# EryiXie/PlaneRecNet

Hardware: AMD Instinct MI355X
Metric: img/s fwd+bwd @480×640 ResNet101-DCN, 1/2/4/8 MI355X + roofline % (higher is better)
Workload: dtype f32 (tensors and accumulation fp32; plain GEMMs and the tap-walked 4x4/s2, 1x1/s2 and sub-pixel convolutions >= 300 tiles: 2xfp16-piece split MFMA, fp32 accumulate; fp32-only rate in fp32_only_run)

## Files before the change

include/prn.h:

```cpp
#ifndef PRN_H
#define PRN_H
#include <stdint.h>
#ifdef __cplusplus
extern "C" {
#endif

#define PRN_BN_SPLITS 32

int prn_version(void);
const char* prn_last_error(void);

enum { PRN_IN_ZERO = 0, PRN_IN_REFLECT = 1, PRN_IN_UP2_REFLECT = 2, PRN_IN_DILATED = 3, PRN_IN_UP2_PHASE = 4,
       PRN_IN_EMBED1 = 5  };
enum { PRN_EPI_NONE = 0, PRN_EPI_RELU = 1, PRN_EPI_SIGMOID = 2 };

enum { PRN_SPLIT_OFF = 0, PRN_SPLIT_PLAN = 1, PRN_SPLIT_ALWAYS = 2 };
enum { PRN_PIECES_BF16 = 0, PRN_PIECES_F16 = 16 };
typedef struct prn_gemm_opts {
  int32_t split_mode;
  int32_t split_kind;
  int32_t split_products;
  int32_t split_min_tiles;
  float split_min_gflop;
  int32_t wgrad_wgs;
// ... 48 lines not shown
typedef struct prn_flip_item {
  const float* src;
  float* dst;
  int M, C, KH, KW;
  int64_t first;
} prn_flip_item;
int prn_weight_flip_transpose_batched(const prn_flip_item* items_dev, int n_items, int64_t total_blocks, void* stream);

int64_t prn_winograd_tiles(int B, int H, int W);
typedef struct prn_winograd_item {
  const float* src;
  float* u;
  float* ut;
  int M, C;
  int64_t first;
} prn_winograd_item;
int prn_winograd_weights_batched(const prn_winograd_item* items_dev, int n_items, int64_t total_blocks, void* stream);
int prn_winograd_input(const float* x, float* V, int B, int C, int H, int W, int in_mode, void* stream);
int64_t prn_gemm_batched_ws_bytes(int M, int C, int P, int nb, const prn_gemm_opts* opts);
int prn_gemm_batched(int M, int C, int P, int nb, const float* U, const void* u_images, const float* V, float* Y, void* ws, const prn_gemm_opts* opts,
                     void* stream);
int prn_winograd_output(const float* Y, const float* bias, const float* addend, float* y, int B, int M, int H, int W, int epilogue, void* stream);
int prn_winograd_output_bn_fwd(const float* Yt, float* x_out, float* stats, const float* gamma, const float* beta, float* y, float* running_mean,
                               float* running_var, int B, int M, int H, int W, float eps, float momentum, int relu, void* stream);
int prn_winograd_output_bn_bwd(const float* Yt, const float* x, const float* stats, const float* gamma, const float* beta, float* dx, float* dgamma,
                               float* dbeta, int B, int M, int H, int W, int relu, void* stream);
int64_t prn_winograd_wgrad_ws_bytes(int B, int C, int H, int W, int M, const prn_gemm_opts* opts);
int prn_winograd_dy(const float* dy, float* Y, int B, int M, int H, int W, void* stream);
int prn_gemm_batched_nt_splits(int M, int C, int P, int nb, const prn_gemm_opts* opts);
int prn_gemm_batched_nt_kind(int M, int C, int P, int nb, const prn_gemm_opts* opts);
int prn_gemm_batched_nt(int M, int C, int P, int nb, const float* A, const float* Bm, float* ws, const prn_gemm_opts* opts, void* stream);
int prn_winograd_dw(const float* partials, float* dw, int M, int C, int splits, void* stream);
int prn_conv3x3_winograd_wgrad(const float* x, const float* dy, float* dw, void* ws, int B, int C, int H, int W, int M, int in_mode, const prn_gemm_opts* opts,
                               void* stream, int phase);
int prn_conv3x3_winograd_wgrad_v(const float* V, const float* dy, float* dw, void* ws, int B, int C, int H, int W, int M, const prn_gemm_opts* opts, void* stream);
int64_t prn_winograd_tiles_ragged(const prn_ragged* rg, int B);
int64_t prn_conv3x3_winograd_ragged_ws_bytes(const prn_ragged* rg, int B, int C, int M, const prn_gemm_opts* opts);
int prn_conv3x3_winograd_ragged(const float* x, const float* U, const void* u_images, const float* bias, const float* addend, float* y, void* ws,
                                const prn_ragged* rg, int B, int C, int M, int epilogue, const prn_gemm_opts* opts, void* stream);
int64_t prn_winograd_wgrad_ragged_ws_bytes(const prn_ragged* rg, int B, int C, int M, const prn_gemm_opts* opts);
int prn_conv3x3_winograd_wgrad_ragged(const float* x, const float* dy, float* dw, void* ws, const prn_ragged* rg, int B, int C, int M, const prn_gemm_opts* opts,
                                      void* stream);
int64_t prn_conv3x3_winograd_ws_bytes(int B, int C, int H, int W, int M, const prn_gemm_opts* opts);
int prn_conv3x3_winograd(const float* x, const float* U, const void* u_images, const float* bias, const float* addend, float* y, void* ws, int B, int C, int H,
                         int W, int M, int in_mode, int epilogue, const prn_gemm_opts* opts, void* stream);

int64_t prn_conv2d_wgrad_ws_bytes(const prn_conv_desc* d);
int prn_conv2d_wgrad_kernel_kind(const prn_conv_desc* d, int G);
int prn_conv2d_wgrad(const prn_conv_desc* d, const float* x, const float* dy, float* dw, void* ws, void* stream);
#define PRN_WGRAD_GROUP_MAX 16
int64_t prn_conv2d_wgrad_grouped_ws_bytes(const prn_conv_desc* d, int G);
int prn_conv2d_wgrad_grouped(const prn_conv_desc* d, int G, const float* const* x, const float* const* dy, float* dw, void* ws, void* stream);
int prn_conv2d_wgrad_phase(const prn_conv_desc* d, const float* x, const float* dy, float* dw, void* ws, void* stream, int phase);

int prn_up2_phase_weights(const float* w, float* wp, int M, int C, void* stream);
int prn_up2_dgrad_weights(const float* w, float* kd, int M, int C, void* stream);
int prn_replicate_fold(const float* dp, float* dx, int B, int C, int H, int W, void* stream);
int prn_space_to_depth2(const float* in, float* out, int B, int C, int H, int W, void* stream);
int prn_up2_wgrad_combine(const float* dwp, float* dw, int M, int C, void* stream);

int prn_pad_fold(const float* dp, float* dx, int B, int C, int H, int W, int up2, void* stream);
int prn_pad_fold_pitched(const float* dp, float* dx, int B, int C, int H, int W, int pitch, void* stream);

int prn_channel_sum(const float* x, float* out, double* ws, int B, int C, int HW, void* stream);

int prn_dcn_sample(const float* x, const float* om, float* cols, int B, int C, int H, int W, int Ho, int Wo,
                   int stride, float max_offset, void* stream);
int64_t prn_dcn_sample_bwd_ws_bytes(int B, int C, int H, int W, int Ho, int Wo);
int prn_dcn_sample_bwd(const float* x, const float* om, const float* dcols, float* dx, float* d_om, void* ws,
                       int B, int C, int H, int W, int Ho, int Wo, int stride, float max_offset, void* stream);

typedef struct prn_dcn_desc {
  int32_t B, C, H, W;
  int32_t M;
  int32_t stride, pad;
  int32_t Ho, Wo;
  int32_t raw;
  float max_offset;
  int32_t epilogue;
  prn_gemm_opts opts;
} prn_dcn_desc;
int64_t prn_dcnv2_table_bytes(const prn_dcn_desc* d);
int prn_dcnv2_table(const prn_dcn_desc* d, const float* offset, const float* mask, void* table, void* stream);
int64_t prn_dcnv2_fwd_ws_bytes(const prn_dcn_desc* d);
int prn_dcnv2_fwd(const prn_dcn_desc* d, const float* x, const void* table, const float* w, const float* bias, float* y, void* ws, void* stream);
int prn_dcnv2_fwd_phase(const prn_dcn_desc* d, const float* x, const void* table, const float* w, const float* bias, float* y, void* ws, void* stream,
                        int phase);
int64_t prn_dcnv2_bwd_weight_ws_bytes(const prn_dcn_desc* d);
int prn_dcnv2_bwd_weight(const prn_dcn_desc* d, const float* x, const void* table, const float* dy, float* dw, void* ws, void* stream);
int prn_dcnv2_bwd_weight_phase(const prn_dcn_desc* d, const float* x, const void* table, const float* dy, float* dw, void* ws, void* stream, int phase);
int64_t prn_dcnv2_bwd_ws_bytes(const prn_dcn_desc* d);
int prn_dcnv2_bwd_input(const prn_dcn_desc* d, const float* dy, const float* wt, const void* wt_images, const float* offset, const float* mask, float* dx,
                        void* ws, void* stream);
int prn_dcnv2_bwd_input_phase(const prn_dcn_desc* d, const float* dy, const float* wt, const void* wt_images, const float* offset, const float* mask,
                              float* dx, void* ws, void* stream, int phase);
int prn_dcnv2_bwd_offset_mask(const prn_dcn_desc* d, const float* x, const float* offset, const float* mask, float* d_offset, float* d_mask,
                              void* ws, void* stream);

int prn_bn_stats(const float* x, float* stats, float* running_mean, float* running_var, double* ws,
                 int B, int C, int HW, float eps, float momentum, void* stream);
int prn_bn_apply(const float* x, const float* stats, const float* gamma, const float* beta, const float* residual,
                 float* y, int B, int C, int HW, int relu, void* stream);
int prn_bn_kernel_kind(int B, int HW);
int prn_bn_train_fwd(const float* x, float* stats, const float* gamma, const float* beta, const float* residual, float* y,
                     float* running_mean, float* running_var, double* ws, int B, int C, int HW, float eps, float momentum,
                     int relu, void* stream);
// ... 188 lines not shown
```

planerecnet_amd/_lib.py:

```python
import ctypes
import os

_HERE = os.path.dirname(os.path.abspath(__file__))
LIB_PATH = os.environ.get("PRN_LIB") or os.path.join(_HERE, "libprn_hip.so")

c_int, c_float, c_void_p, c_i64 = ctypes.c_int, ctypes.c_float, ctypes.c_void_p, ctypes.c_int64


class GemmOpts(ctypes.Structure):
    _fields_ = [("split_mode", ctypes.c_int32), ("split_kind", ctypes.c_int32), ("split_products", ctypes.c_int32), ("split_min_tiles", ctypes.c_int32),
                ("split_min_gflop", ctypes.c_float), ("wgrad_wgs", ctypes.c_int32), ("wgrad_target", ctypes.c_int32), ("wgrad_split", ctypes.c_int32)]

    def key(self):
        return (self.split_mode, self.split_kind, self.split_products, self.split_min_tiles, self.split_min_gflop, self.wgrad_wgs, self.wgrad_target, self.wgrad_split)


SPLIT_OFF, SPLIT_PLAN, SPLIT_ALWAYS = 0, 1, 2
PIECES_BF16, PIECES_F16 = 0, 16


class ConvDesc(ctypes.Structure):
    _fields_ = [(n, ctypes.c_int32) for n in
                ("B", "C", "H", "W", "M", "KH", "KW", "stride", "pad", "Ho", "Wo", "in_mode", "dil", "epilogue", "ystride", "yH", "yW", "reserved")] + [
                    ("opts", GemmOpts)]
# ... 27 lines not shown
P = c_void_p
_DP = ctypes.POINTER(ConvDesc)
_OP = ctypes.POINTER(GemmOpts)
SIGNATURES = {
    "prn_version": (c_int, []),
    "prn_last_error": (ctypes.c_char_p, []),
    "prn_conv2d_fwd_ws_bytes": (c_i64, [_DP]),
    "prn_conv2d_kernel_kind": (c_int, [_DP]),
    "prn_conv2d_fwd_partials": (c_int, [_DP, ctypes.POINTER(c_i64)]),
    "prn_gemm_opts_default": (None, [_OP]),
    "prn_gemm_pipe": (c_int, [c_int, c_int, c_int, c_int, c_int, _OP]),
    "prn_split_images_bytes": (c_i64, [c_int, c_int, c_int]),
    "prn_split_prepare": (c_int, [P, P, c_int, c_int, c_int, c_int, P]),
    "prn_split_prepare_batched": (c_int, [P, c_int, c_i64, c_i64, c_int, P]),
    "prn_conv2d_fwd": (c_int, [_DP, P, P, P, P, P, P, P]),
    "prn_conv2d_fwd_ragged": (c_int, [_DP, P, P, P, P, P, P, P]),
    "prn_conv2d_wgrad_ragged_ws_bytes": (c_i64, [_DP, P]),
    "prn_conv2d_wgrad_ragged": (c_int, [_DP, P, P, P, P, P, P]),
    "prn_gn_relu_fwd_ragged": (c_int, [P, P, P, P, P, c_int, c_int, c_int, P, c_int, c_float, P]),
    "prn_gn_relu_bwd_ragged": (c_int, [P, P, P, P, P, P, P, P, c_int, c_int, c_int, P, c_int, P]),
    "prn_conv2d_fwd_phase": (c_int, [_DP, P, P, P, P, P, P, P, c_int]),
    "prn_conv2d_fwd_counted": (c_int, [_DP, P, P, P, P, P, P, P, P, P, c_int]),
    "prn_conv2d_wgrad_phase": (c_int, [_DP, P, P, P, P, P, c_int]),
    "prn_weight_flip_transpose": (c_int, [P, P, c_int, c_int, c_int, c_int, P]),
    "prn_weight_flip_transpose_batched": (c_int, [P, c_int, c_i64, P]),
    "prn_winograd_tiles": (c_i64, [c_int, c_int, c_int]),
    "prn_winograd_weights_batched": (c_int, [P, c_int, c_i64, P]),
    "prn_winograd_input": (c_int, [P, P, c_int, c_int, c_int, c_int, c_int, P]),
    "prn_gemm_batched_ws_bytes": (c_i64, [c_int, c_int, c_int, c_int, _OP]),
    "prn_gemm_batched": (c_int, [c_int, c_int, c_int, c_int, P, P, P, P, P, _OP, P]),
    "prn_winograd_output": (c_int, [P, P, P, P, c_int, c_int, c_int, c_int, c_int, P]),
    "prn_winograd_output_bn_fwd": (c_int, [P] * 8 + [c_int] * 4 + [c_float, c_float, c_int, P]),
    "prn_winograd_output_bn_bwd": (c_int, [P] * 8 + [c_int] * 5 + [P]),
    "prn_winograd_wgrad_ws_bytes": (c_i64, [c_int] * 5 + [_OP]),
    "prn_winograd_dy": (c_int, [P, P, c_int, c_int, c_int, c_int, P]),
    "prn_gemm_batched_nt_splits": (c_int, [c_int] * 4 + [_OP]),
    "prn_gemm_batched_nt_kind": (c_int, [c_int] * 4 + [_OP]),
    "prn_conv2d_wgrad_kernel_kind": (c_int, [_DP, c_int]),
    "prn_gemm_batched_nt": (c_int, [c_int, c_int, c_int, c_int, P, P, P, _OP, P]),
    "prn_winograd_dw": (c_int, [P, P, c_int, c_int, c_int, P]),
    "prn_conv3x3_winograd_wgrad": (c_int, [P, P, P, P, c_int, c_int, c_int, c_int, c_int, c_int, _OP, P, c_int]),
    "prn_winograd_tiles_ragged": (c_i64, [P, c_int]),
    "prn_conv3x3_winograd_ragged_ws_bytes": (c_i64, [P, c_int, c_int, c_int, _OP]),
    "prn_conv3x3_winograd_ragged": (c_int, [P, P, P, P, P, P, P, P, c_int, c_int, c_int, c_int, _OP, P]),
    "prn_winograd_wgrad_ragged_ws_bytes": (c_i64, [P, c_int, c_int, c_int, _OP]),
    "prn_conv3x3_winograd_wgrad_ragged": (c_int, [P, P, P, P, P, c_int, c_int, c_int, _OP, P]),
    "prn_conv3x3_winograd_wgrad_v": (c_int, [P, P, P, P, c_int, c_int, c_int, c_int, c_int, _OP, P]),
    "prn_conv3x3_winograd_ws_bytes": (c_i64, [c_int] * 5 + [_OP]),
    "prn_conv3x3_winograd": (c_int, [P, P, P, P, P, P, P, c_int, c_int, c_int, c_int, c_int, c_int, c_int, _OP, P]),
    "prn_conv2d_wgrad_ws_bytes": (c_i64, [_DP]),
    "prn_conv2d_wgrad_grouped_ws_bytes": (c_i64, [_DP, c_int]),
    "prn_conv2d_wgrad_grouped": (c_int, [_DP, c_int, P, P, P, P, P]),
    "prn_conv2d_wgrad": (c_int, [_DP, P, P, P, P, P]),
    "prn_pad_fold": (c_int, [P, P, c_int, c_int, c_int, c_int, c_int, P]),
    "prn_pad_fold_pitched": (c_int, [P, P, c_int, c_int, c_int, c_int, c_int, P]),
    "prn_up2_phase_weights": (c_int, [P, P, c_int, c_int, P]),
    "prn_up2_dgrad_weights": (c_int, [P, P, c_int, c_int, P]),
    "prn_up2_wgrad_combine": (c_int, [P, P, c_int, c_int, P]),
    "prn_space_to_depth2": (c_int, [P, P, c_int, c_int, c_int, c_int, P]),
    "prn_replicate_fold": (c_int, [P, P, c_int, c_int, c_int, c_int, P]),
    "prn_channel_sum": (c_int, [P, P, P, c_int, c_int, c_int, P]),
    "prn_dcn_sample": (c_int, [P, P, P] + [c_int] * 7 + [c_float, P]),
    "prn_dcn_sample_bwd_ws_bytes": (c_i64, [c_int] * 6),
    "prn_dcn_sample_bwd": (c_int, [P, P, P, P, P, P] + [c_int] * 7 + [c_float, P]),
    "prn_dcnv2_table_bytes": (c_i64, [P]),
    "prn_dcnv2_table": (c_int, [P, P, P, P, P]),
    "prn_dcnv2_fwd_ws_bytes": (c_i64, [P]),
    "prn_dcnv2_fwd": (c_int, [P] * 8),
    "prn_dcnv2_fwd_phase": (c_int, [P] * 8 + [c_int]),
    "prn_dcnv2_bwd_weight_ws_bytes": (c_i64, [P]),
    "prn_dcnv2_bwd_weight": (c_int, [P] * 7),
    "prn_dcnv2_bwd_weight_phase": (c_int, [P] * 7 + [c_int]),
    "prn_dcnv2_bwd_ws_bytes": (c_i64, [P]),
    "prn_dcnv2_bwd_input": (c_int, [P] * 9),
    "prn_dcnv2_bwd_input_phase": (c_int, [P] * 9 + [c_int]),
    "prn_bn_kernel_kind": (c_int, [c_int, c_int]),
    "prn_dcnv2_bwd_offset_mask": (c_int, [P] * 8),
    "prn_plane_prior_ws_bytes": (c_i64, [c_int] * 6 + [_OP]),
    "prn_plane_prior_fwd": (c_int, [P] * 7 + [c_int] * 6 + [_OP, P]),
    "prn_plane_prior_fwd_phase": (c_int, [P] * 7 + [c_int] * 6 + [_OP, P, c_int]),
    "prn_plane_prior_wgrad_ws_bytes": (c_i64, [c_int] * 5 + [_OP]),
    "prn_plane_prior_wgrad": (c_int, [P] * 4 + [c_int] * 5 + [_OP, P]),
    "prn_fpn_level_ws_bytes": (c_i64, [c_int] * 8 + [_OP]),
    "prn_fpn_level_fwd": (c_int, [P, P, P, P, c_int, c_int, P, P, P, P, P, P] + [c_int] * 6 + [_OP, P]),
    "prn_frame_to_input": (c_int, [P] + [c_int] * 6 + [P, P, c_int, P, P, P]),
    "prn_mask_loss_ws_floats": (c_int, [c_int]),
    "prn_mask_loss_fwd": (c_int, [P] * 9 + [c_int, c_int, c_int, c_float, c_float, P]),
    "prn_mask_loss_bwd": (c_int, [P] * 8 + [c_int, c_int, P]),
    "prn_vnl_triplets": (c_int, [P] * 12 + [c_int, c_int, c_int, c_float, P]),
    "prn_vnl_scatter": (c_int, [P] * 5 + [c_int, c_int, P]),
    "prn_depth_metrics_ws_doubles": (c_int, []),
    "prn_depth_metrics": (c_int, [P, P, P, P, c_i64, c_float, c_float, P]),
    "prn_vnl_trim_key": (c_int, [P, P, P, P, c_int, P]),
    "prn_vnl_trim_fwd": (c_int, [P, P, P, P, P, P, P, c_int, c_int, c_int, P, P, P, P, P, P]),
    "prn_vnl_trim_ws_bytes": (c_i64, [c_int]),
    "prn_vnl_trim_bwd": (c_int, [P, P, P, P, P, P, P, c_int, c_int, P, P]),
    "prn_loss_ws_doubles": (c_int, [c_int]),
    "prn_focal_sum_fwd": (c_int, [P, P, P, P, c_i64, c_int, c_float, c_float, P]),
    "prn_focal_sum_bwd": (c_int, [P, P, P, P, c_i64, c_int, c_float, c_float, P]),
    "prn_rmse_log_fwd": (c_int, [P, P, P, P, P, c_int, c_int, c_float, c_float, P]),
    "prn_rmse_log_bwd": (c_int, [P, P, P, P, P, c_int, c_int, c_float, c_float, P]),
    "prn_gt_segments": (c_i64, [c_int, c_int]),
    "prn_gt_mask_stats": (c_int, [P, P, c_int, c_int, c_int, c_int, P, P, P, P]),
    "prn_gt_quarter_masks": (c_int, [P, P, c_int, c_int, c_int, P]),
    "prn_gt_sample_triplets": (c_int, [P, P, c_int, c_int, c_int, c_int, P, P, P, P, P, ctypes.c_uint64, ctypes.c_uint64, c_i64, P, P]),
    "prn_adam_chunk_elems": (c_int, []),
# ... 73 lines not shown
```

planerecnet_amd/losses.py:

```python
import collections
import os
import threading

import numpy as np
import torch
import torch.nn.functional as F
from torch import nn

from . import ops
from .config import cfg
from .funcs import center_of_mass, quarter_mask_u8


def _pin(x):
    return x.pin_memory()


class Targets:
    __slots__ = ("B", "cell_ids", "cell_gidx", "cell_inv", "cells_unique", "n_pos", "n_pos_dev", "pos_img", "ins_labels", "cate_labels", "num_ins", "vnl", "lava_adj", "lava_gsum",
                 "ready")


LOSS_STREAMS = bool(int(os.environ.get("PRN_LOSS_STREAMS", "0")))

# ... 108 lines not shown
                "cell_inv": pin(torch.from_numpy(cell_inv)) if cell_mult > 1 else None,
                "cells_unique": cell_mult <= 2,
                "cell_ids": pin(torch.from_numpy(np.concatenate(cell_ids))), "pos_img": pin(torch.from_numpy(np.repeat(np.arange(B), n_pos))),
                "ins_labels": pin(torch.cat(ins_labels, 0)),
                "cate_labels": pin(torch.cat([r for lv in range(L) for r in cate_rows[lv]])),
                "vnl": (self.vnl.prepare_host(host, (H, W)) if cfg.use_plane_loss else None) if with_vnl else "deferred"}

    @torch.no_grad()
    def upload(self, h, gt_depths, device):
        t = Targets()
        t.ready = None
        t.B, t.n_pos, t.num_ins = h["B"], h["n_pos"], h["num_ins"]
        up = lambda x: x.to(device, non_blocking=True)
        t.cell_ids = list(up(h["cell_ids"]).split(h["n_pos"]))
        t.cell_gidx, t.cells_unique = up(h["cell_gidx"]), h["cells_unique"]
        t.cell_inv = up(h["cell_inv"]) if h["cell_inv"] is not None else None
        t.n_pos_dev = up(h["n_pos_f"])
        t.pos_img, t.ins_labels, t.cate_labels = up(h["pos_img"]), up(h["ins_labels"]), up(h["cate_labels"])
        t.vnl = self.vnl.upload(h["vnl"], device) if h["vnl"] is not None else None
        t.lava_gsum = t.lava_adj = None
        if cfg.use_lava_loss:
            B, (H, W), (fh, fw) = h["B"], h["hw"], h["feat"]
            if gt_depths.is_cuda and gt_depths.dtype == torch.float32 and LAVA_GT_KERNEL:
                gd = gt_depths.contiguous()
                grad = torch.empty_like(gd)
                ops.check(ops.lib.prn_lava_gt_weights(ops._p(gd), ops._p(grad), B, H, W, float(self.depth_resolution), ops._stream()), "prn_lava_gt_weights")
                t.lava_gsum = ops.channel_sum(grad.view(1, B, H, W))
            else:
                grad = sobel_sq(gt_depths) / gt_depths.clamp(min=self.depth_resolution) ** 2
                grad = grad.clamp(max=1e-2)
                grad = torch.where(grad < 1e-4, torch.zeros_like(grad), grad)
                t.lava_gsum = grad.flatten(1).sum(1)
            adj = torch.empty(B, 1, fh, fw, device=device, dtype=torch.float32)
            ops.check(ops.lib.prn_resize_bilinear_bwd(ops._p(grad.contiguous()), ops._p(adj), B, fh, fw, H, W, ops._stream()), "prn_resize_bilinear_bwd")
            t.lava_adj = adj
        return t

    def prepare(self, gt_instances, gt_depths, device, mask_feat_size=None):
        return self.upload(self.prepare_host(gt_instances, tuple(gt_depths.shape[-2:]), mask_feat_size), gt_depths, device)

    def forward(self, net, mask_preds, cate_preds, kernel_preds, depth_preds, gt_instances, gt_depths, targets=None):
        dev = mask_preds.device
        B = mask_preds.shape[0]
        fh, fw = mask_preds.shape[-2:]
        t = targets if targets is not None else self.prepare(gt_instances, gt_depths, dev, (fh, fw))
        if getattr(t, "ready", None) is not None:
            torch.cuda.current_stream().wait_event(t.ready)
            t.ready = None
        E = kernel_preds[0].shape[1]

        def instance_terms():
            out = {}
            flat_k = torch.cat([k.reshape(B, E, -1) for k in kernel_preds], 2)
            preds = []
            per_image = torch.split(mask_preds, 1)
            if t.cells_unique and sum(t.n_pos) > 0:
                rows = flat_k.transpose(1, 2).reshape(B * flat_k.shape[2], E).index_select(0, t.cell_gidx)
                if t.cell_inv is not None:
                    rows = rows.index_select(0, t.cell_inv)
                w_img = [r.reshape(-1, E, 1, 1) for r in torch.split(rows, t.n_pos)]
            else:
                flat_kb = flat_k.unbind(0)
                w_img = [flat_kb[b][:, t.cell_ids[b]].t().reshape(t.n_pos[b], E, 1, 1).contiguous() if t.n_pos[b] else None for b in range(B)]
            for b in range(B):
                if t.n_pos[b] == 0:
                    continue
                preds.append(ops.conv2d(per_image[b], w_img[b]).view(t.n_pos[b], fh, fw))
            logits = torch.cat(preds, 0)
            if FUSED_LOSS and logits.is_cuda and logits.shape[0] > 0 and (fh * fw) % 4 == 0 and B <= 64:
                lava = cfg.use_lava_loss
                ins, lav = _MaskLoss.apply(logits, t.ins_labels, t.pos_img, t.lava_adj if lava else None, t.lava_gsum if lava else None,
                                           t.n_pos_dev if lava else None, float(self.ins_loss_weight), float(self.lava_loss_weight))
                out["ins"] = ins
                if lava:
                    out["lav"] = lav
                return out
            ins_sig = torch.sigmoid(logits)
            out["ins"] = dice_loss(ins_sig, t.ins_labels).mean() * self.ins_loss_weight
            if cfg.use_lava_loss:
                seg, npos = t.pos_img, t.n_pos_dev
                num = torch.zeros(B, device=dev, dtype=ins_sig.dtype).index_add_(0, seg, (ins_sig * t.lava_adj[seg, 0]).flatten(1).sum(1))
                ok = (t.lava_gsum > 0) & (npos > 0)
                per_img = torch.where(ok, num / (t.lava_gsum * npos).clamp(min=1e-30), torch.zeros_like(num))
                out["lav"] = per_img.sum() / ok.sum().clamp(min=1) * self.lava_loss_weight
            return out

        def category_term():
            flat_pred = torch.cat([c.permute(0, 2, 3, 1).reshape(-1, self.num_classes) for c in cate_preds])
            if FUSED_LOSS and FUSED_CAT_DPT and flat_pred.is_cuda:
                return {"cat": self.conf_loss_weight * _FocalSum.apply(flat_pred, t.cate_labels, self.focal_loss_alpha, self.focal_loss_gamma) / (t.num_ins + 1)}
            onehot = F.one_hot(t.cate_labels, self.num_classes + 1)[:, : self.num_classes].to(flat_pred.dtype)
            return {"cat": self.conf_loss_weight * sigmoid_focal_sum(flat_pred, onehot, self.focal_loss_alpha, self.focal_loss_gamma) / (t.num_ins + 1)}

        def depth_terms():
            dp = ops.resize_bilinear(depth_preds, (2 * depth_preds.shape[2], 2 * depth_preds.shape[3]))
            if FUSED_LOSS and FUSED_CAT_DPT and dp.is_cuda:
                out = {"dpt": self.depth_loss_weight * _RmseLog.apply(dp, gt_depths, cfg.dataset.min_depth, 1e-9)}
            else:
                out = {"dpt": self.depth_loss_weight * rmse_log(dp, gt_depths, gt_depths > cfg.dataset.min_depth)}
            if cfg.use_plane_loss:
                out["pln"] = self.vnl.batched(dp, gt_depths, t.vnl).mean() * self.pln_loss_weight
            return out

        parts = ops.run_branches([instance_terms, category_term, depth_terms]) if (LOSS_STREAMS and mask_preds.is_cuda) else \
            [instance_terms(), category_term(), depth_terms()]
        losses = {}
        for part in parts:
            losses.update(part)
        if all(k in losses for k in ("ins", "cat", "dpt", "pln", "lav")):
            losses = {k: losses[k] for k in ("ins", "cat", "dpt", "pln", "lav")}
        return losses


FUSED_CAT_DPT = bool(int(os.environ.get("PRN_FUSED_CAT_DPT", "1")))
FUSED_LOSS = bool(int(os.environ.get("PRN_FUSED_LOSS", "1")))


class _MaskLoss(torch.autograd.Function):

    @staticmethod
    def forward(ctx, logits, labels, pos_img, adj, gsum, npos, w_ins, w_lav):
        logits, labels = logits.contiguous(), labels.contiguous()
        P, HW = logits.shape[0], logits[0].numel()
        B = adj.shape[0] if adj is not None else 1
        dev = logits.device
        out = torch.empty(2, device=dev, dtype=torch.float32)
        coef = torch.empty(P, 3, device=dev, dtype=torch.float32)
        ws = torch.empty(ops.lib.prn_mask_loss_ws_floats(P), device=dev, dtype=torch.float32)
        adj_c = adj.contiguous() if adj is not None else None
        ops.check(ops.lib.prn_mask_loss_fwd(ops._p(logits), ops._p(labels), ops._p(adj_c), ops._p(pos_img), ops._p(gsum), ops._p(npos), ops._p(out),
                                            ops._p(coef), ops._p(ws), P, HW, B, w_ins, w_lav, ops._stream()), "prn_mask_loss_fwd")
        ctx.save_for_backward(logits, labels, pos_img, adj_c, coef)
        ins, lav = out.unbind(0)
        return ins, lav

    @staticmethod
    def backward(ctx, g_ins, g_lav):
        logits, labels, pos_img, adj, coef = ctx.saved_tensors
        dz = torch.empty_like(logits)
        g_ins = None if g_ins is None else g_ins.contiguous().float()
        g_lav = None if g_lav is None else g_lav.contiguous().float()
        ops.check(ops.lib.prn_mask_loss_bwd(ops._p(logits), ops._p(labels), ops._p(adj), ops._p(pos_img), ops._p(coef), ops._p(g_ins), ops._p(g_lav),
                                            ops._p(dz), logits.shape[0], logits[0].numel(), ops._stream()), "prn_mask_loss_bwd")
        return dz, None, None, None, None, None, None, None


def dice_loss(p, t):
    p = p.reshape(p.shape[0], -1)
    t = t.reshape(t.shape[0], -1).float()
    return 1 - 2 * (p * t).sum(1) / ((p * p).sum(1) + 0.001 + (t * t).sum(1) + 0.001)


def sigmoid_focal_sum(x, t, alpha, gamma):
    p = torch.sigmoid(x)
    ce = F.binary_cross_entropy_with_logits(x, t, reduction="none")
    p_t = p * t + (1 - p) * (1 - t)
    loss = ce * (1 - p_t) ** gamma
    if alpha >= 0:
        loss = (alpha * t + (1 - alpha) * (1 - t)) * loss
    return loss.sum()


def rmse_log(pred, gt, valid, clamp=1e-9):
    n = pred.shape[0]
    l1 = (torch.log(pred.reshape(n, -1).clamp(min=clamp)) - torch.log(gt.reshape(n, -1).clamp(min=clamp))).abs().mul(valid.reshape(n, -1))
    return torch.sqrt((l1 ** 2).sum(1) / valid.reshape(n, -1).sum(1)).mean()
# ... 590 lines not shown
```

planerecnet_amd/ops.py:

```python
import ctypes

import os
import threading
import weakref

import torch

from . import _lib, profiling
from ._lib import ConvDesc, GemmOpts, IN_ZERO, IN_REFLECT, IN_UP2_REFLECT, IN_DILATED, IN_UP2_PHASE, IN_EMBED1, EPI_NONE, EPI_RELU, EPI_SIGMOID, lib, check


_SIDE = {}
WGRAD_ASYNC = bool(int(os.environ.get("PRN_WGRAD_ASYNC", "0")))


WGRAD_WGS_ASYNC = os.environ.get("PRN_WGRAD_WGS_ASYNC", "512")


_POLICY = {"split_mode": int(os.environ.get("PRN_SPLIT_GEMM", "1")),
           "kind": _lib.PIECES_BF16 if os.environ.get("PRN_SPLIT_KIND", "f16") == "bf16" else _lib.PIECES_F16,
           "products": int(os.environ.get("PRN_SPLIT16_PRODUCTS", "3")),
           "min_gflop": float(os.environ.get("PRN_SPLIT_MIN_GFLOP", "4.0")),
           "min_tiles": int(os.environ.get("PRN_SPLIT_MIN_TILES", os.environ.get("PRN_SPLIT_MIN_TILES_EVAL", "300"))),
           "wgrad_wgs": int(os.environ.get("PRN_WGRAD_WGS", "0") or 0),
# ... 993 lines not shown


class _ConvUp2(torch.autograd.Function):

    @staticmethod
    def forward(ctx, x, w, bias):
        _dev(x, w, bias)
        bias_param = bias
        x, w, bias = _c(x), _c(w), _c(bias)
        B, C, H, W = x.shape
        M = w.shape[0]
        assert w.shape[1:] == (C, 3, 3), (x.shape, w.shape)
        wp = torch.empty(4, M, C, 2, 2, device=x.device, dtype=torch.float32)
        check(lib.prn_up2_phase_weights(_p(w), _p(wp), M, C, _stream()), "prn_up2_phase_weights")
        y = conv_fwd_raw(x, wp, bias, None, M, 2, 1, 0, 2 * H, 2 * W, IN_UP2_PHASE)
        ctx.save_for_backward(x, w)
        ctx.has_bias = bias is not None
        ctx.bias = bias_param
        return y

    @staticmethod
    def backward(ctx, dy):
        x, w = ctx.saved_tensors
        dy = _c(dy)
        B, C, H, W = x.shape
        M = w.shape[0]
        dx = dw = db = None
        if ctx.needs_input_grad[0]:
            kd = torch.empty(C, M, 4, 4, device=x.device, dtype=torch.float32)
            check(lib.prn_up2_dgrad_weights(_p(w), _p(kd), M, C, _stream()), "prn_up2_dgrad_weights")
            dp = conv_fwd_raw(dy, kd, None, None, C, 4, 2, 3, H + 2, W + 2)
            dx = torch.empty_like(x)
            check(lib.prn_replicate_fold(_p(dp), _p(dx), B, C, H, W, _stream()), "prn_replicate_fold")
        def wgrad():
            dyp = torch.empty(4, B, M, H, W, device=x.device, dtype=torch.float32)
            check(lib.prn_space_to_depth2(_p(dy), _p(dyp), B, M, H, W, _stream()), "prn_space_to_depth2")
            dwp = conv_wgrad_raw(x, dyp, M, 2, 1, 0, IN_UP2_PHASE)
            dwo = torch.empty_like(w)
            check(lib.prn_up2_wgrad_combine(_p(dwp), _p(dwo), M, C, _stream()), "prn_up2_wgrad_combine")
            if getattr(_TLS, "side", None) is not None:
                _HELD.append((dyp, dwp))
            return dwo
        if _defer(ctx.needs_input_grad[1], w):
            _deferred_wgrad(w, (x, dy), wgrad, fast=True)
        elif ctx.needs_input_grad[1]:
            dw = wgrad()
        db = _bias_grad(ctx.has_bias and ctx.needs_input_grad[2], ctx.bias, dy)
        return dx, dw, db


UP2_SUBPIXEL = bool(int(os.environ.get("PRN_UP2_SUBPIXEL", "1")))


def conv2d(x, w, bias=None, stride=1, pad=0, in_mode=IN_ZERO, epilogue=EPI_NONE, addend=None):
    if in_mode == IN_UP2_REFLECT and UP2_SUBPIXEL and epilogue == EPI_NONE and addend is None and x.shape[2] > 1 and x.shape[3] > 1:
        return _ConvUp2.apply(x, w, bias)
    return _Conv2d.apply(x, w, bias, addend, stride, pad, in_mode, epilogue, False)


_UP2_PHASE = {}


def conv_up2_inference(x, w, bias=None, relu=False):
    _dev(x, w, bias)
    x, w, bias = _c(x), _c(w), _c(bias)
    B, C, H, W = x.shape
    M = w.shape[0]
    assert w.shape[1:] == (C, 3, 3), (x.shape, w.shape)
    if not (UP2_SUBPIXEL and H > 1 and W > 1):
        return conv2d(x, w, bias, 1, 1, IN_UP2_REFLECT, EPI_RELU if relu else EPI_NONE)
    e = _UP2_PHASE.get(w.data_ptr())
    if e is None or e[0]() is not w or e[1] != w._version:
        wp = torch.empty(4, M, C, 2, 2, device=x.device, dtype=torch.float32)
        check(lib.prn_up2_phase_weights(_p(w), _p(wp), M, C, _stream()), "prn_up2_phase_weights")
        ptr = w.data_ptr()
        e = _UP2_PHASE[ptr] = (weakref.ref(w), w._version, wp)
        weakref.finalize(w, lambda p=ptr, r=e[0]: _UP2_PHASE.pop(p, None) if (_UP2_PHASE.get(p) or (None,))[0] is r else None)
    return conv_fwd_raw(x, e[2], bias, None, M, 2, 1, 0, 2 * H, 2 * W, IN_UP2_PHASE, 1, EPI_RELU if relu else EPI_NONE)


def conv2d_fork(x, w, bias=None, stride=1, pad=0, in_mode=IN_ZERO, epilogue=EPI_NONE, addend=None):
    return _Conv2d.apply(x, w, bias, addend, stride, pad, in_mode, epilogue, True)


_DCN = {}


def _dcn_desc(B, C, H, W, M, stride, pad, raw, max_offset, epi=EPI_NONE):
    oe = _opts_entry("colgrad" in SPLIT_SKIP)
    key = (B, C, H, W, M, stride, pad, raw, float(max_offset), epi, oe[2])
    e = _DCN.get(key)
    if e is None:
        Ho, Wo = (H + 2 * pad - 3) // stride + 1, (W + 2 * pad - 3) // stride + 1
        d = _lib.DcnDesc(B, C, H, W, M, stride, pad, Ho, Wo, int(raw), float(max_offset), epi, oe[0])
        ref = ctypes.byref(d)
        sizes = [lib.prn_dcnv2_table_bytes(ref), lib.prn_dcnv2_fwd_ws_bytes(ref), lib.prn_dcnv2_bwd_weight_ws_bytes(ref), lib.prn_dcnv2_bwd_ws_bytes(ref)]
        if min(sizes) < 0:
            raise RuntimeError(lib.prn_last_error().decode())
        e = _DCN[key] = (d, ref, sizes[0], sizes[1], sizes[2], sizes[3])
    return e


def _f32(nbytes, dev):
    return torch.empty(max(nbytes // 4, 1), device=dev, dtype=torch.float32)


# ... 685 lines not shown
```

Before: 193.8.

## Batch per-image mask dynamic convolutions into one ragged grouped GEMM kernel

Replaces the per-image loop of 1x1 conv2d calls that apply predicted instance kernels to mask features with a single ragged grouped GEMM. New HIP kernels cover forward, dgrad and a split-K wgrad with a reduce pass, reading a per-image row/block table from kernel arguments, so there is one launch per pass instead of one per image plus a cat. It uses plain fp32 MFMA 32x32x2 rather than the split fp16 path, and falls back to the old loop when the plan helper rejects the shapes.

```diff
diff --git a/include/prn.h b/include/prn.h
--- a/include/prn.h
+++ b/include/prn.h
@@ -124,6 +124,13 @@
 int64_t prn_conv2d_wgrad_grouped_ws_bytes(const prn_conv_desc* d, int G);
 int prn_conv2d_wgrad_grouped(const prn_conv_desc* d, int G, const float* const* x, const float* const* dy, float* dw, void* ws, void* stream);
 int prn_conv2d_wgrad_phase(const prn_conv_desc* d, const float* x, const float* dy, float* dw, void* ws, void* stream, int phase);
+
+#define PRN_DYNCONV_MAX_IMAGES 32
+int prn_dynconv_fwd(const float* feat, const float* rows, float* logits, int B, int E, int HW, const int* n_rows, const int* splits, void* stream);
+int prn_dynconv_dgrad(const float* rows, const float* dlogits, float* dfeat, int B, int E, int HW, const int* n_rows, const int* splits, void* stream);
+int64_t prn_dynconv_wgrad_ws_bytes(int B, int E, const int* n_rows, const int* splits);
+int prn_dynconv_wgrad(const float* dlogits, const float* feat, float* drows, void* ws, int B, int E, int HW, const int* n_rows, const int* splits,
+                      void* stream, int phase);
 
 int prn_up2_phase_weights(const float* w, float* wp, int M, int C, void* stream);
 int prn_up2_dgrad_weights(const float* w, float* kd, int M, int C, void* stream);
diff --git a/planerecnet_amd/_lib.py b/planerecnet_amd/_lib.py
--- a/planerecnet_amd/_lib.py
+++ b/planerecnet_amd/_lib.py
@@ -103,6 +103,10 @@
     "prn_conv2d_wgrad_grouped_ws_bytes": (c_i64, [_DP, c_int]),
     "prn_conv2d_wgrad_grouped": (c_int, [_DP, c_int, P, P, P, P, P]),
     "prn_conv2d_wgrad": (c_int, [_DP, P, P, P, P, P]),
+    "prn_dynconv_fwd": (c_int, [P, P, P, c_int, c_int, c_int, P, P, P]),
+    "prn_dynconv_dgrad": (c_int, [P, P, P, c_int, c_int, c_int, P, P, P]),
+    "prn_dynconv_wgrad_ws_bytes": (c_i64, [c_int, c_int, P, P]),
+    "prn_dynconv_wgrad": (c_int, [P, P, P, P, c_int, c_int, c_int, P, P, P, c_int]),
     "prn_pad_fold": (c_int, [P, P, c_int, c_int, c_int, c_int, c_int, P]),
     "prn_pad_fold_pitched": (c_int, [P, P, c_int, c_int, c_int, c_int, c_int, P]),
     "prn_up2_phase_weights": (c_int, [P, P, c_int, c_int, P]),
diff --git a/planerecnet_amd/csrc/prn_dynconv.hip b/planerecnet_amd/csrc/prn_dynconv.hip
--- /dev/null
+++ b/planerecnet_amd/csrc/prn_dynconv.hip
@@ -0,0 +1,292 @@
+#include <stddef.h>
+#include "prn_common.h"
+
+typedef float f32x16 __attribute__((ext_vector_type(16)));
+
+namespace {
+
+constexpr int MAXB = PRN_DYNCONV_MAX_IMAGES;
+struct Tab {
+  int nimg;
+  int row0[MAXB + 1];
+  int blk0[MAXB + 1];
+  int splits[MAXB];
+  int wso[MAXB + 1];
+};
+struct DynArgs {
+  const float* a; const float* b; float* out;
+  int E, HW;
+  Tab tab;
+};
+__device__ __forceinline__ int tab_read(size_t member_offset, int i) {
+  typedef __attribute__((address_space(4))) const int* kptr;
+  kptr base = (kptr)__builtin_amdgcn_kernarg_segment_ptr();
+  return base[(offsetof(DynArgs, tab) + member_offset) / 4 + i];
+}
+#define TAB(member, i) tab_read(offsetof(Tab, member), i)
+
+__device__ __forceinline__ int find_image(int nimg, int bid) {
+  int img = 0;
+  for (int t = 1; t < nimg; ++t)
+    if (bid >= TAB(blk0, t)) img = t;
+  return img;
+}
+
+enum { DYN_FWD = 0, DYN_DGRAD = 1, DYN_WGRAD = 2 };
+
+template <int MODE>
+__global__ __launch_bounds__(256) void dynconv_kernel(DynArgs a) {
+  constexpr int BK = 16, LD = BK + 1, NE = BK / 4;
+  constexpr bool A_KFAST = MODE != DYN_DGRAD;
+  constexpr bool B_KFAST = MODE == DYN_WGRAD;
+  __shared__ float As[2][64 * LD];
+  __shared__ float Bs[2][B_KFAST ? 64 * LD : BK * 64];
+  const int tid = threadIdx.x, lane = tid & 63, wave = tid >> 6;
+  const int wm = wave >> 1, wn = wave & 1;
+  const int bid = blockIdx.x;
+  const int img = find_image(a.tab.nimg, bid);
+  const int r0 = TAB(row0, img), n = TAB(row0, img + 1) - r0, S = TAB(splits, img);
+  const int lid = bid - TAB(blk0, img);
+  const int E = a.E, HW = a.HW;
+
+  int m0, j0, Mlim, Jlim, K, split = 0;
+  if (MODE == DYN_FWD) {
+    const int tm = (n + 63) >> 6;
+    m0 = (lid % tm) * 64; j0 = (lid / tm) * 64; Mlim = n; Jlim = HW; K = E;
+  } else if (MODE == DYN_DGRAD) {
+    const int tm = (E + 63) >> 6;
+    m0 = (lid % tm) * 64; j0 = (lid / tm) * 64; Mlim = E; Jlim = HW; K = n;
+  } else {
+    const int tm = (n + 63) >> 6, nt = tm * ((E + 63) >> 6);
+    const int tile = lid % nt;
+    split = lid / nt;
+    m0 = (tile % tm) * 64; j0 = (tile / tm) * 64; Mlim = n; Jlim = E; K = HW;
+  }
+  const int T = (K + 15) >> 4;
+  const int kt_begin = MODE == DYN_WGRAD ? (int)((int64_t)split * T / S) : 0, kt_end = MODE == DYN_WGRAD ? (int)((int64_t)(split + 1) * T / S) : T;
+  const bool rows_here = m0 + wm * 32 < Mlim;
+
+  const int ak = A_KFAST ? (tid & 15) : (tid >> 6), am = A_KFAST ? (tid >> 4) : (tid & 63);
+  const int bk = B_KFAST ? (tid & 15) : (tid >> 6), bj = B_KFAST ? (tid >> 4) : (tid & 63);
+  const float* ap; const float* bp;
+  int a_ms, a_ks, b_js, b_ks;
+  if (MODE == DYN_FWD) {
+    ap = a.a + (size_t)r0 * E; a_ms = E; a_ks = 1;
+    bp = a.b + (size_t)img * E * HW; b_js = 1; b_ks = HW;
+  } else if (MODE == DYN_DGRAD) {
+    ap = a.a + (size_t)r0 * E; a_ms = 1; a_ks = E;
+    bp = a.b + (size_t)r0 * HW; b_js = 1; b_ks = HW;
+  } else {
+    ap = a.a + (size_t)r0 * HW; a_ms = HW; a_ks = 1;
+    bp = a.b + (size_t)img * E * HW; b_js = HW; b_ks = 1;
+  }
+
+  float ra[NE], rb[NE];
+  auto load_slice = [&](int kt) {
+    const int k0 = kt * 16, kend = kt < kt_end ? K : 0;
+#pragma unroll
+    for (int i = 0; i < NE; ++i) {
+      const int m = m0 + am + (A_KFAST ? 16 * i : 0), k = k0 + ak + (A_KFAST ? 0 : 4 * i);
+      const bool ok = m < Mlim && k < kend;
+      ra[i] = ok ? ap[(size_t)m * a_ms + (size_t)k * a_ks] : 0.f;
+    }
+#pragma unroll
+    for (int i = 0; i < NE; ++i) {
+      const int j = j0 + bj + (B_KFAST ? 16 * i : 0), k = k0 + bk + (B_KFAST ? 0 : 4 * i);
+      const bool ok = j < Jlim && k < kend;
+      rb[i] = ok ? bp[(size_t)j * b_js + (size_t)k * b_ks] : 0.f;
+    }
+  };
+  auto store_slice = [&](int buf) {
+#pragma unroll
+    for (int i = 0; i < NE; ++i) As[buf][(am + (A_KFAST ? 16 * i : 0)) * LD + ak + (A_KFAST ? 0 : 4 * i)] = ra[i];
+#pragma unroll
+    for (int i = 0; i < NE; ++i) {
+      if (B_KFAST) Bs[buf][(bj + 16 * i) * LD + bk] = rb[i];
+      else Bs[buf][(bk + 4 * i) * 64 + bj] = rb[i];
+    }
+  };
+  f32x16 acc, tot;
+#pragma unroll
+  for (int r = 0; r < 16; ++r) { acc[r] = 0.f; tot[r] = 0.f; }
+  auto mma_slice = [&](int buf) {
+    if (!rows_here) return;
+#pragma unroll
+    for (int kk = 0; kk < BK / 2; ++kk) {
+      const int k = kk * 2 + (lane >> 5);
+      const float av = As[buf][(wm * 32 + (lane & 31)) * LD + k];
+      const float bv = B_KFAST ? Bs[buf][(wn * 32 + (lane & 31)) * LD + k] : Bs[buf][k * 64 + wn * 32 + (lane & 31)];
+      acc = __builtin_amdgcn_mfma_f32_32x32x2f32(av, bv, acc, 0, 0, 0);
+    }
+  };
+
+  const bool fold = MODE != DYN_WGRAD && S > 1;
+  int sp = 0, bnd = fold ? (int)((int64_t)T / S) : -1;
+  while (fold && bnd <= 0 && sp < S - 1) { ++sp; bnd = (int)((int64_t)(sp + 1) * T / S); }
+  load_slice(kt_begin);
+  int buf = 0;
+  for (int kt = kt_begin; kt < kt_end; ++kt) {
+    store_slice(buf);
+    __syncthreads();
+    load_slice(kt + 1);
+    mma_slice(buf);
+    buf ^= 1;
+    if (fold && kt + 1 == bnd) {
+#pragma unroll
+      for (int r = 0; r < 16; ++r) { tot[r] += acc[r]; acc[r] = 0.f; }
+      do { ++sp; bnd = (int)((int64_t)(sp + 1) * T / S); } while (bnd <= kt + 1 && sp < S - 1);
+    }
+  }
+  if (fold) acc = tot;
+  float* outp;
+  int ldo;
+  if (MODE == DYN_WGRAD) {
+    outp = a.out + (size_t)TAB(wso, img) + (size_t)split * n * E;
+    ldo = E;
+  } else {
+    outp = MODE == DYN_FWD ? a.out + (size_t)r0 * HW : a.out + (size_t)img * E * HW;
+    ldo = HW;
+  }
+  const int j = j0 + wn * 32 + (lane & 31);
+  if (j >= Jlim) return;
+#pragma unroll
+  for (int r = 0; r < 16; ++r) {
+    const int m = m0 + wm * 32 + (r & 3) + 8 * (r >> 2) + 4 * (lane >> 5);
+    if (m < Mlim) outp[(size_t)m * ldo + j] = acc[r];
+  }
+}
+
+__global__ __launch_bounds__(256) void dynconv_reduce_kernel(DynArgs a) {
+  __shared__ float sm[4][64];
+  const int bid = blockIdx.x;
+  const int img = find_image(a.tab.nimg, bid);
+  const int r0 = TAB(row0, img), n = TAB(row0, img + 1) - r0, splits = TAB(splits, img);
+  const int64_t cnt = (int64_t)n * a.E;
+  const float* ws = a.a + (size_t)TAB(wso, img);
+  const int e = threadIdx.x & 63, g = threadIdx.x >> 6;
+  const int64_t i = (int64_t)(bid - TAB(blk0, img)) * 64 + e;
+  float acc = 0.f;
+  if (i < cnt) {
+    float a0 = 0.f, a1 = 0.f, a2 = 0.f, a3 = 0.f;
+    int k = g;
+    for (; k + 12 < splits; k += 16) {
+      a0 += ws[(size_t)k * cnt + i];
+      a1 += ws[(size_t)(k + 4) * cnt + i];
+      a2 += ws[(size_t)(k + 8) * cnt + i];
+      a3 += ws[(size_t)(k + 12) * cnt + i];
+    }
+    for (; k < splits; k += 4) a0 += ws[(size_t)k * cnt + i];
+    acc = (a0 + a1) + (a2 + a3);
+  }
+  sm[g][e] = acc;
+  __syncthreads();
+  if (g == 0 && i < cnt) a.out[(size_t)r0 * a.E + i] = (sm[0][e] + sm[1][e]) + (sm[2][e] + sm[3][e]);
+}
+
+int check_common(const char* who, int B, int E, int HW, const int* n_rows, const int* splits, int64_t* N) {
+  PRN_REQUIRE(B >= 1 && B <= MAXB, "%s: 1 <= B <= %d images (got %d)", who, MAXB, B);
+  PRN_REQUIRE(E >= 1 && HW >= 1, "%s: empty dimension", who);
+  PRN_REQUIRE(n_rows != nullptr && splits != nullptr, "%s: null row-count / split table", who);
+  int64_t total = 0;
+  for (int b = 0; b < B; ++b) {
+    PRN_REQUIRE(n_rows[b] >= 0, "%s: negative row count for image %d", who, b);
+    PRN_REQUIRE(n_rows[b] == 0 || (splits[b] >= 1 && splits[b] <= 4096), "%s: image %d: split count %d out of range", who, b, splits[b]);
+    total += n_rows[b];
+  }
+  PRN_REQUIRE(total * HW < (1LL << 31) && (int64_t)B * E * HW < (1LL << 31) && total * E < (1LL << 31), "%s: tensor too large for 32-bit indexing", who);
+  *N = total;
+  return 0;
+}
+
+void fill_rows(Tab& t, int B, const int* n_rows, const int* splits) {
+  t.nimg = B;
+  int r = 0;
+  for (int b = 0; b < MAXB; ++b) {
+    t.row0[b] = r;
+    if (b < B) r += n_rows[b];
+    t.splits[b] = (b < B && n_rows[b] > 0) ? splits[b] : 1;
+    t.blk0[b] = 0; t.wso[b] = 0;
+  }
+  t.row0[MAXB] = r; t.blk0[MAXB] = 0; t.wso[MAXB] = 0;
+}
+
+}
+
+extern "C" int prn_dynconv_fwd(const float* feat, const float* rows, float* logits, int B, int E, int HW, const int* n_rows, const int* splits, void* stream) {
+  int64_t N = 0;
+  if (int e = check_common("prn_dynconv_fwd", B, E, HW, n_rows, splits, &N)) return e;
+  if (N == 0) return 0;
+  PRN_REQUIRE(feat && rows && logits, "prn_dynconv_fwd: null tensor");
+  DynArgs a;
+  a.a = rows; a.b = feat; a.out = logits; a.E = E; a.HW = HW;
+  fill_rows(a.tab, B, n_rows, splits);
+  int64_t blocks = 0;
+  for (int b = 0; b <= MAXB; ++b) {
+    a.tab.blk0[b] = (int)blocks;
+    if (b < B) blocks += (int64_t)cdiv(n_rows[b], 64) * cdiv(HW, 64);
+  }
+  PRN_REQUIRE(blocks < (1LL << 31), "prn_dynconv_fwd: too many tiles");
+  hipLaunchKernelGGL((dynconv_kernel<DYN_FWD>), dim3((unsigned)blocks), dim3(256), 0, (hipStream_t)stream, a);
+  PRN_CHECK_LAUNCH("prn_dynconv_fwd");
+  return 0;
+}
+
+extern "C" int prn_dynconv_dgrad(const float* rows, const float* dlogits, float* dfeat, int B, int E, int HW, const int* n_rows, const int* splits,
+                                 void* stream) {
+  int64_t N = 0;
+  if (int e = check_common("prn_dynconv_dgrad", B, E, HW, n_rows, splits, &N)) return e;
+  PRN_REQUIRE(dfeat && (N == 0 || (rows && dlogits)), "prn_dynconv_dgrad: null tensor");
+  DynArgs a;
+  a.a = rows; a.b = dlogits; a.out = dfeat; a.E = E; a.HW = HW;
+  fill_rows(a.tab, B, n_rows, splits);
+  const int64_t per = (int64_t)cdiv(E, 64) * cdiv(HW, 64);
+  for (int b = 0; b <= MAXB; ++b) a.tab.blk0[b] = (int)(per * (b < B ? b : B));
+  PRN_REQUIRE(per * B < (1LL << 31), "prn_dynconv_dgrad: too many tiles");
+  hipLaunchKernelGGL((dynconv_kernel<DYN_DGRAD>), dim3((unsigned)(per * B)), dim3(256), 0, (hipStream_t)stream, a);
+  PRN_CHECK_LAUNCH("prn_dynconv_dgrad");
+  return 0;
+}
+
+extern "C" int64_t prn_dynconv_wgrad_ws_bytes(int B, int E, const int* n_rows, const int* splits) {
+  if (B < 1 || B > MAXB || E < 1 || n_rows == nullptr || splits == nullptr) { prn_set_error("prn_dynconv_wgrad_ws_bytes: bad arguments"); return -1; }
+  int64_t floats = 0;
+  for (int b = 0; b < B; ++b) {
+    if (n_rows[b] < 0 || (n_rows[b] > 0 && splits[b] < 1)) { prn_set_error("prn_dynconv_wgrad_ws_bytes: bad row / split count for image %d", b); return -1; }
+    floats += (int64_t)n_rows[b] * E * (n_rows[b] > 0 ? splits[b] : 0);
+  }
+  return floats * 4;
+}
+
+extern "C" int prn_dynconv_wgrad(const float* dlogits, const float* feat, float* drows, void* ws, int B, int E, int HW, const int* n_rows, const int* splits,
+                                 void* stream, int phase) {
+  int64_t N = 0;
+  if (int e = check_common("prn_dynconv_wgrad", B, E, HW, n_rows, splits, &N)) return e;
+  if (N == 0) return 0;
+  PRN_REQUIRE(dlogits && feat && drows && ws, "prn_dynconv_wgrad: null tensor / workspace (prn_dynconv_wgrad_ws_bytes)");
+  PRN_REQUIRE(prn_dynconv_wgrad_ws_bytes(B, E, n_rows, splits) < (1LL << 33), "prn_dynconv_wgrad: workspace beyond 32-bit element offsets");
+  DynArgs a;
+  a.a = dlogits; a.b = feat; a.out = (float*)ws; a.E = E; a.HW = HW;
+  fill_rows(a.tab, B, n_rows, splits);
+  DynArgs r = a;
+  r.a = (const float*)ws; r.b = nullptr; r.out = drows;
+  int64_t blocks = 0, rblocks = 0, wso = 0;
+  for (int b = 0; b <= MAXB; ++b) {
+    a.tab.blk0[b] = (int)blocks; r.tab.blk0[b] = (int)rblocks;
+    a.tab.wso[b] = r.tab.wso[b] = (int)wso;
+    if (b < B && n_rows[b] > 0) {
+      blocks += (int64_t)cdiv(n_rows[b], 64) * cdiv(E, 64) * splits[b];
+      rblocks += cdiv((int64_t)n_rows[b] * E, 64);
+      wso += (int64_t)n_rows[b] * E * splits[b];
+    }
+  }
+  PRN_REQUIRE(blocks < (1LL << 31) && wso < (1LL << 31), "prn_dynconv_wgrad: too many tiles");
+  if (phase != 2) {
+    hipLaunchKernelGGL((dynconv_kernel<DYN_WGRAD>), dim3((unsigned)blocks), dim3(256), 0, (hipStream_t)stream, a);
+    PRN_CHECK_LAUNCH("prn_dynconv_wgrad");
+  }
+  if (phase != 1) {
+    hipLaunchKernelGGL(dynconv_reduce_kernel, dim3((unsigned)rblocks), dim3(256), 0, (hipStream_t)stream, r);
+    PRN_CHECK_LAUNCH("prn_dynconv_wgrad/reduce");
+  }
+  return 0;
+}
diff --git a/planerecnet_amd/losses.py b/planerecnet_amd/losses.py
--- a/planerecnet_amd/losses.py
+++ b/planerecnet_amd/losses.py
@@ -184,21 +184,22 @@
         def instance_terms():
             out = {}
             flat_k = torch.cat([k.reshape(B, E, -1) for k in kernel_preds], 2)
-            preds = []
-            per_image = torch.split(mask_preds, 1)
-            if t.cells_unique and sum(t.n_pos) > 0:
+            any_pos = sum(t.n_pos) > 0
+            if t.cells_unique and any_pos:
                 rows = flat_k.transpose(1, 2).reshape(B * flat_k.shape[2], E).index_select(0, t.cell_gidx)
                 if t.cell_inv is not None:
                     rows = rows.index_select(0, t.cell_inv)
-                w_img = [r.reshape(-1, E, 1, 1) for r in torch.split(rows, t.n_pos)]
+            if MASK_DYNCONV and t.cells_unique and mask_preds.is_cuda and (not any_pos or ops.dynconv_plans(t.n_pos, E, fh, fw) is not None):
+                logits = ops.mask_dynconv(mask_preds, rows, t.n_pos) if any_pos else mask_preds.new_empty((0, fh, fw))
             else:
-                flat_kb = flat_k.unbind(0)
-                w_img = [flat_kb[b][:, t.cell_ids[b]].t().reshape(t.n_pos[b], E, 1, 1).contiguous() if t.n_pos[b] else None for b in range(B)]
-            for b in range(B):
-                if t.n_pos[b] == 0:
-                    continue
-                preds.append(ops.conv2d(per_image[b], w_img[b]).view(t.n_pos[b], fh, fw))
-            logits = torch.cat(preds, 0)
+                per_image = torch.split(mask_preds, 1)
+                if t.cells_unique and any_pos:
+                    w_img = [r.reshape(-1, E, 1, 1) for r in torch.split(rows, t.n_pos)]
+                else:
+                    flat_kb = flat_k.unbind(0)
+                    w_img = [flat_kb[b][:, t.cell_ids[b]].t().reshape(t.n_pos[b], E, 1, 1).contiguous() if t.n_pos[b] else None for b in range(B)]
+                preds = [ops.conv2d(per_image[b], w_img[b]).view(t.n_pos[b], fh, fw) for b in range(B) if t.n_pos[b]]
+                logits = torch.cat(preds, 0)
             if FUSED_LOSS and logits.is_cuda and logits.shape[0] > 0 and (fh * fw) % 4 == 0 and B <= 64:
                 lava = cfg.use_lava_loss
                 ins, lav = _MaskLoss.apply(logits, t.ins_labels, t.pos_img, t.lava_adj if lava else None, t.lava_gsum if lava else None,
@@ -244,6 +245,7 @@
         return losses
 
 
+MASK_DYNCONV = bool(int(os.environ.get("PRN_MASK_DYNCONV", "1")))
 FUSED_CAT_DPT = bool(int(os.environ.get("PRN_FUSED_CAT_DPT", "1")))
 FUSED_LOSS = bool(int(os.environ.get("PRN_FUSED_LOSS", "1")))
 
diff --git a/planerecnet_amd/ops.py b/planerecnet_amd/ops.py
--- a/planerecnet_amd/ops.py
+++ b/planerecnet_amd/ops.py
@@ -1069,6 +1069,92 @@
 UP2_SUBPIXEL = bool(int(os.environ.get("PRN_UP2_SUBPIXEL", "1")))
 
 
+DYNCONV_MAX_IMAGES = 32
+
+
+def dynconv_plans(n_rows, E, H, W):
+    B = len(n_rows)
+    if B > DYNCONV_MAX_IMAGES:
+        return None
+    f, g, w = [1] * B, [1] * B, [1] * B
+    for b, n in enumerate(n_rows):
+        if n == 0:
+            continue
+        for out, (C, M) in ((f, (E, n)), (g, (n, E))):
+            d, _, fb, _, parts = _desc(1, C, H, W, M, 1, 1, 0, H, W)
+            if d.kind != 0 or (parts is None and fb):
+                return None
+            out[b] = parts[0] if parts is not None else 1
+        _, ref, _, wb, _ = _desc(1, E, H, W, n, 1, 1, 0, H, W)
+        if lib.prn_conv2d_wgrad_kernel_kind(ref, 1) != 0:
+            return None
+        w[b] = wb // (4 * n * E) if wb else 1
+    arr = ctypes.c_int * B
+    return arr(*f), arr(*g), arr(*w)
+
+
+def _dynconv_plans_or_raise(n_rows, E, H, W):
+    plans = dynconv_plans(n_rows, E, H, W)
+    if plans is None:
+        raise RuntimeError("mask_dynconv: the launch policy changed between forward and backward (see ops.dynconv_plans)")
+    return plans
+
+
+class _MaskDynConv(torch.autograd.Function):
+    @staticmethod
+    def forward(ctx, feat, rows, n_rows):
+        _dev(feat, rows)
+        feat, rows = _c(feat), _c(rows)
+        B, E, H, W = feat.shape
+        N, HW = rows.shape[0], H * W
+        assert N == sum(n_rows) and rows.shape[1] == E and len(n_rows) == B, (feat.shape, rows.shape, n_rows)
+        logits = torch.empty(N, H, W, device=feat.device, dtype=torch.float32)
+        nr = (ctypes.c_int * B)(*n_rows)
+        sp = _dynconv_plans_or_raise(n_rows, E, H, W)[0]
+        with profiling.span("conv_igemm_kernel", "mfma", 2.0 * N * E * HW, nbytes=4.0 * (feat.numel() + rows.numel() + logits.numel()), tag=("dynconv", E, H, W, N, B)):
+            check(lib.prn_dynconv_fwd(_p(feat), _p(rows), _p(logits), B, E, HW, nr, sp, _stream()), "prn_dynconv_fwd")
+        ctx.save_for_backward(feat, rows)
+        ctx.n_rows = tuple(n_rows)
+        return logits
+
+    @staticmethod
+    def backward(ctx, dlogits):
+        feat, rows = ctx.saved_tensors
+        n_rows = ctx.n_rows
+        B, E, H, W = feat.shape
+        N, HW = rows.shape[0], H * W
+        dlogits = _c(dlogits)
+        nr = (ctypes.c_int * B)(*n_rows)
+        _, sg, sw = _dynconv_plans_or_raise(n_rows, E, H, W)
+        dfeat = drows = None
+        fl = 2.0 * N * E * HW
+        prof = profiling._enabled
+        if ctx.needs_input_grad[0]:
+            dfeat = torch.empty_like(feat)
+            with profiling.span("conv_igemm_kernel", "mfma", fl, nbytes=4.0 * (feat.numel() + rows.numel() + dlogits.numel()), tag=("dynconv_dgrad", E, H, W, N, B)):
+                check(lib.prn_dynconv_dgrad(_p(rows), _p(dlogits), _p(dfeat), B, E, HW, nr, sg, _stream()), "prn_dynconv_dgrad")
+        if ctx.needs_input_grad[1]:
+            drows = torch.empty_like(rows)
+            nbytes = lib.prn_dynconv_wgrad_ws_bytes(B, E, nr, sw)
+            if nbytes < 0:
+                raise RuntimeError(lib.prn_last_error().decode())
+            ws = _wspace(nbytes, feat.device)
+            if prof:
+                with profiling.span("conv_wgrad_kernel", "mfma", fl, nbytes=4.0 * (feat.numel() + rows.numel() + dlogits.numel()), tag=("dynconv_wgrad", E, H, W, N, B)):
+                    check(lib.prn_dynconv_wgrad(_p(dlogits), _p(feat), _p(drows), _p(ws), B, E, HW, nr, sw, _stream(), 1), "prn_dynconv_wgrad")
+                with profiling.span("reduce_splits_kernel", "hbm", float(nbytes) + 4.0 * drows.numel()):
+                    check(lib.prn_dynconv_wgrad(_p(dlogits), _p(feat), _p(drows), _p(ws), B, E, HW, nr, sw, _stream(), 2), "prn_dynconv_wgrad")
+            else:
+                check(lib.prn_dynconv_wgrad(_p(dlogits), _p(feat), _p(drows), _p(ws), B, E, HW, nr, sw, _stream(), 0), "prn_dynconv_wgrad")
+        return dfeat, drows, None
+
+
+def mask_dynconv(feat, rows, n_rows):
+    if rows.shape[0] == 0:
+        return feat.new_empty((0,) + tuple(feat.shape[2:]))
+    return _MaskDynConv.apply(feat, rows, tuple(int(n) for n in n_rows))
+
+
 def conv2d(x, w, bias=None, stride=1, pad=0, in_mode=IN_ZERO, epilogue=EPI_NONE, addend=None):
     if in_mode == IN_UP2_REFLECT and UP2_SUBPIXEL and epilogue == EPI_NONE and addend is None and x.shape[2] > 1 and x.shape[3] > 1:
         return _ConvUp2.apply(x, w, bias)
```

Result: no change. 195.4, median of 6 (+0.8%).
